# pythoncrazy/jimm

Hardware: NVIDIA H100
Metric: images/sec (higher is better)
Workload: dtype f16

## Files before the change

### jimm_b200/csrc/attention.cu

```cuda
#include <cmath>
#include <type_traits>

#include "common.cuh"
#include "kernels.cuh"

namespace jimm {

__device__ __forceinline__ void cp_async_commit() { asm volatile("cp.async.commit_group;" ::); }
template <int N>
__device__ __forceinline__ void cp_async_wait() { asm volatile("cp.async.wait_group %0;" ::"n"(N)); }

template <typename T>
__device__ __forceinline__ uint32_t pack_pair(float a, float b) {
  if constexpr (std::is_same<T, __half>::value) {
    __half2 h = __floats2half2_rn(a, b);
    return *reinterpret_cast<uint32_t*>(&h);
  } else {
    __nv_bfloat162 h = __floats2bfloat162_rn(a, b);
    return *reinterpret_cast<uint32_t*>(&h);
  }
}

static constexpr int QT = 64;
static constexpr int KT = 64;

template <int DP>
struct HeadTile {
  static_assert(DP % 16 == 0 && DP >= 16 && DP <= 128, "padded head width");
  static constexpr int ROWB = DP * 2;
  static constexpr int SW = ROWB % 128 == 0 ? 128 : ROWB % 64 == 0 ? 64 : 32;
  static constexpr int NB = ROWB / SW;
  static constexpr int CH = SW / 16;
  static constexpr int NCH = DP / 8;
  static constexpr int BYTES = QT * ROWB;
  static constexpr int SMEM = 5 * BYTES;
  static __device__ __forceinline__ uint32_t off(uint32_t row, uint32_t ch) {
    const uint32_t blk = ch / CH, cb = ch % CH;
    return blk * (QT * SW) + row * SW + ((cb ^ ((row * SW >> 7) & (CH - 1))) << 4);
  }
  static __device__ __forceinline__ uint64_t kstep(int ks) { return static_cast<uint64_t>(((ks * 32) / SW * (QT * SW) + (ks * 32) % SW) >> 4); }
};

__device__ __forceinline__ void cp_async16_zfill(uint32_t dst, const void* src, uint32_t src_bytes) {
  asm volatile("cp.async.cg.shared.global [%0], [%1], 16, %2;" ::"r"(dst), "l"(src), "r"(src_bytes));
}

template <typename T, int DP>
__device__ __forceinline__ void load_tile(uint32_t smem_base, const T* __restrict__ gbase, size_t ld, int s0, int S, int d, int tid) {
  using L = HeadTile<DP>;
#pragma unroll
  for (int i = 0; i < L::NCH * QT / 128; ++i) {
    const uint32_t c = tid + i * 128;
    const uint32_t row = c / L::NCH, ch = c % L::NCH;
    int s = s0 + static_cast<int>(row);
    s = s < S ? s : S - 1;
    const bool in = static_cast<int>(ch * 8) < d;
    const T* src = gbase + static_cast<size_t>(s) * ld + (in ? ch * 8 : 0);
    cp_async16_zfill(smem_base + L::off(row, ch), src, in ? 16u : 0u);
  }
}

template <int BYTES, bool STATIC = (BYTES <= 48 * 1024)>
struct AttnSmem {
  static __device__ __forceinline__ uint8_t* get() {
    __shared__ __align__(1024) uint8_t smem[BYTES];
    return smem;
  }
};
template <int BYTES>
struct AttnSmem<BYTES, false> {
  static __device__ __forceinline__ uint8_t* get() {
    extern __shared__ uint8_t smem_raw[];
    return reinterpret_cast<uint8_t*>((reinterpret_cast<uintptr_t>(smem_raw) + 1023) & ~static_cast<uintptr_t>(1023));
  }
};

template <bool PACKED>
__device__ __forceinline__ void sample_rows(int b, int S_arg, const int* __restrict__ seq_off, size_t& row0, int& S) {
  if constexpr (PACKED) {
    row0 = static_cast<size_t>(seq_off[b]);
    S = seq_off[b + 1] - seq_off[b];
  } else {
    row0 = static_cast<size_t>(b) * S_arg;
    S = S_arg;
  }
}

template <typename T, int DP>
__device__ __forceinline__ void score_tile(float (&s)[8][4], uint64_t qdesc, uint32_t sK) {
  using L = HeadTile<DP>;
  constexpr bool BF16 = std::is_same<T, __nv_bfloat16>::value;
  float (&s_acc)[32] = reinterpret_cast<float (&)[32]>(s);
  const uint64_t kdesc = make_wgmma_desc<L::SW>(sK, 16);
#pragma unroll
  for (int i = 0; i < 32; ++i) s_acc[i] = 0.f;
  wgmma_fence_operands(s_acc);
  wgmma_fence();
#pragma unroll
  for (int ks = 0; ks < DP / 16; ++ks)
    wgmma_m64n64k16_ss<BF16>(s_acc, qdesc + L::kstep(ks), kdesc + L::kstep(ks), ks != 0 ? 1u : 0u);
  wgmma_commit();
  wgmma_wait<0>();
  wgmma_fence_operands(s_acc);
}

template <bool CAUSAL>
__device__ __forceinline__ void mask_tile(float (&s)[8][4], int k0, int q0, int row_lo, int t4, int S) {
  if ((k0 + KT > S) || (CAUSAL && (k0 + KT - 1 > q0))) {
#pragma unroll
    for (int nt = 0; nt < 8; ++nt) {
#pragma unroll
      for (int e = 0; e < 4; ++e) {
        const int key = k0 + nt * 8 + t4 * 2 + (e & 1);
        const int qrow = row_lo + (e >> 1) * 8;
        const bool ok = key < S && (!CAUSAL || key <= qrow);
        if (!ok) s[nt][e] = -INFINITY;
      }
    }
  }
}

__device__ __forceinline__ float2 softmax_step(float (&s)[8][4], float (&m_run)[2], float (&l_run)[2], float scale_log2) {
  float mx[2] = {-INFINITY, -INFINITY};
#pragma unroll
  for (int nt = 0; nt < 8; ++nt) {
    mx[0] = fmaxf(mx[0], fmaxf(s[nt][0], s[nt][1]));
    mx[1] = fmaxf(mx[1], fmaxf(s[nt][2], s[nt][3]));
  }
  float alpha[2], moff[2];
#pragma unroll
  for (int r = 0; r < 2; ++r) {
    mx[r] = fmaxf(mx[r], __shfl_xor_sync(0xffffffffu, mx[r], 1));
    mx[r] = fmaxf(mx[r], __shfl_xor_sync(0xffffffffu, mx[r], 2));
    const float mnew = fmaxf(m_run[r], mx[r]);
    const float muse = (mnew == -INFINITY) ? 0.f : mnew;
    alpha[r] = exp2f((m_run[r] - muse) * scale_log2);
    m_run[r] = mnew;
    moff[r] = muse * scale_log2;
    l_run[r] *= alpha[r];
  }
#pragma unroll
  for (int nt = 0; nt < 8; ++nt) {
    s[nt][0] = exp2f(s[nt][0] * scale_log2 - moff[0]);
    s[nt][1] = exp2f(s[nt][1] * scale_log2 - moff[0]);
    s[nt][2] = exp2f(s[nt][2] * scale_log2 - moff[1]);
    s[nt][3] = exp2f(s[nt][3] * scale_log2 - moff[1]);
    l_run[0] += s[nt][0] + s[nt][1];
    l_run[1] += s[nt][2] + s[nt][3];
  }
  return make_float2(alpha[0], alpha[1]);
}

__device__ __forceinline__ float row_inv_sum(float l) {
  l += __shfl_xor_sync(0xffffffffu, l, 1);
  l += __shfl_xor_sync(0xffffffffu, l, 2);
  return 1.0f / l;
}

template <typename T, typename OutT, bool CAUSAL, int DP, bool PACKED = false>
__global__ void __launch_bounds__(128)
attention_kernel(const T* __restrict__ qkv, OutT* __restrict__ out, int S_arg, int H, int d, float scale_log2, int reverse,
                 const int* __restrict__ seq_off) {
  using L = HeadTile<DP>;
  uint8_t* smem = AttnSmem<L::SMEM>::get();
  const int tid = threadIdx.x, warp = tid >> 5, lane = tid & 31;
  const int qt = blockIdx.x, h = blockIdx.y, b = reverse ? static_cast<int>(gridDim.z) - 1 - static_cast<int>(blockIdx.z) : static_cast<int>(blockIdx.z);
  const int D = H * d;
  const size_t ld = static_cast<size_t>(3) * D;
  if constexpr (PACKED) {
    pdl_launch_dependents();
    pdl_wait();
  }
  size_t row0;
  int S;
  sample_rows<PACKED>(b, S_arg, seq_off, row0, S);
  if (PACKED && qt * QT >= S) return;
  const T* base = qkv + row0 * ld + h * d;
  const T* gq = base;
  const T* gk = base + D;
  const T* gv = base + 2 * D;
  const uint32_t sQ = smem_u32(smem);
  const uint32_t sK0 = sQ + L::BYTES;
  const uint32_t sV0 = sK0 + 2 * L::BYTES;
  const int q0 = qt * QT;
  if constexpr (!PACKED) {
    pdl_launch_dependents();
    pdl_wait();
  }
  int n_kv = (S + KT - 1) / KT;
  if (CAUSAL) n_kv = min(n_kv, qt + 1);

  load_tile<T, DP>(sQ, gq, ld, q0, S, d, tid);
  load_tile<T, DP>(sK0, gk, ld, 0, S, d, tid);
  load_tile<T, DP>(sV0, gv, ld, 0, S, d, tid);
  cp_async_commit();

  constexpr bool BF16 = std::is_same<T, __nv_bfloat16>::value;
  const uint64_t qdesc = make_wgmma_desc<L::SW>(sQ, 16);
  float o[DP / 8][4];
#pragma unroll
  for (int i = 0; i < DP / 8; ++i)
#pragma unroll
    for (int j = 0; j < 4; ++j) o[i][j] = 0.f;
  float m_run[2] = {-INFINITY, -INFINITY}, l_run[2] = {0.f, 0.f};
  const int g = lane >> 2, t4 = lane & 3;
  const int row_lo = q0 + warp * 16 + g;

  for (int j = 0; j < n_kv; ++j) {
    const int buf = j & 1;
    if (j + 1 < n_kv) {
      load_tile<T, DP>(sK0 + (buf ^ 1) * L::BYTES, gk, ld, (j + 1) * KT, S, d, tid);
      load_tile<T, DP>(sV0 + (buf ^ 1) * L::BYTES, gv, ld, (j + 1) * KT, S, d, tid);
      cp_async_commit();
      cp_async_wait<1>();
    } else {
      cp_async_wait<0>();
    }
    fence_proxy_async_smem();
    __syncthreads();
    const uint32_t sK = sK0 + buf * L::BYTES, sV = sV0 + buf * L::BYTES;

    float s[8][4];
    score_tile<T, DP>(s, qdesc, sK);
    mask_tile<CAUSAL>(s, j * KT, q0, row_lo, t4, S);
    const float2 alpha = softmax_step(s, m_run, l_run, scale_log2);
#pragma unroll
    for (int nt = 0; nt < DP / 8; ++nt) {
      o[nt][0] *= alpha.x; o[nt][1] *= alpha.x;
      o[nt][2] *= alpha.y; o[nt][3] *= alpha.y;
    }
    uint32_t pf[4][4];
#pragma unroll
    for (int kk = 0; kk < 4; ++kk) {
      pf[kk][0] = pack_pair<T>(s[2 * kk][0], s[2 * kk][1]);
      pf[kk][1] = pack_pair<T>(s[2 * kk][2], s[2 * kk][3]);
      pf[kk][2] = pack_pair<T>(s[2 * kk + 1][0], s[2 * kk + 1][1]);
      pf[kk][3] = pack_pair<T>(s[2 * kk + 1][2], s[2 * kk + 1][3]);
    }
    float (&o_acc)[DP / 2] = reinterpret_cast<float (&)[DP / 2]>(o);
    const uint64_t vdesc = make_wgmma_desc<L::SW>(sV, L::NB > 1 ? QT * L::SW : 16);
    wgmma_fence_operands(o_acc);
    wgmma_fence();
#pragma unroll
    for (int kk = 0; kk < 4; ++kk) wgmma_m64nNk16_rs<BF16, DP>(o_acc, pf[kk], vdesc + static_cast<uint64_t>(kk * (16 * L::SW >> 4)));
    wgmma_commit();
    wgmma_wait<0>();
    wgmma_fence_operands(o_acc);
    __syncthreads();
  }

  const float inv[2] = {row_inv_sum(l_run[0]), row_inv_sum(l_run[1])};
  OutT* obase = out + row0 * D + h * d;
  if constexpr (sizeof(OutT) == 2) {
    uint8_t* sq = smem;
#pragma unroll
    for (int nt = 0; nt < DP / 8; ++nt) {
#pragma unroll
      for (int r = 0; r < 2; ++r) {
        const int row = warp * 16 + g + r * 8;
        const int ch = nt;
        const uint32_t v = pack_pair<OutT>(o[nt][2 * r] * inv[r], o[nt][2 * r + 1] * inv[r]);
        *reinterpret_cast<uint32_t*>(sq + L::off(row, ch) + t4 * 4) = v;
      }
    }
    __syncwarp();
#pragma unroll
    for (int i = 0; i < L::NCH / 2; ++i) {
      const uint32_t c = i * 32 + lane;
      const int row = warp * 16 + static_cast<int>(c / L::NCH), ch = static_cast<int>(c % L::NCH);
      const int srow = q0 + row;
      if (srow < S && ch * 8 < d) {
        const uint4 v = *reinterpret_cast<const uint4*>(sq + L::off(row, ch));
        *reinterpret_cast<uint4*>(obase + static_cast<size_t>(srow) * D + ch * 8) = v;
      }
    }
  } else {
#pragma unroll
    for (int nt = 0; nt < DP / 8; ++nt) {
      if (nt * 8 >= d) break;
#pragma unroll
      for (int r = 0; r < 2; ++r) {
        const int srow = row_lo + r * 8;
        if (srow < S) {
          float2 v = make_float2(o[nt][2 * r] * inv[r], o[nt][2 * r + 1] * inv[r]);
          if constexpr (std::is_same<OutT, tf32_t>::value) v = make_float2(round_tf32(v.x), round_tf32(v.y));
          *reinterpret_cast<float2*>(reinterpret_cast<float*>(obase) + static_cast<size_t>(srow) * D + nt * 8 + t4 * 2) = v;
        }
      }
    }
  }
}

static int padded_head_dim(int d) { return d <= 16 ? 16 : d <= 32 ? 32 : d <= 64 ? 64 : d <= 80 ? 80 : d <= 96 ? 96 : 128; }

static float attn_scale_log2(int d) { return static_cast<float>(1.0 / std::sqrt(static_cast<double>(d))) * 1.4426950408889634f; }

template <typename F>
static int attn_variant(int d, int causal, const int* seq_off, F&& f) {
  auto at_width = [&](auto c, auto p) -> int {
    switch (padded_head_dim(d)) {
      case 16: return f(c, std::integral_constant<int, 16>{}, p);
      case 32: return f(c, std::integral_constant<int, 32>{}, p);
      case 64: return f(c, std::integral_constant<int, 64>{}, p);
      case 80: return f(c, std::integral_constant<int, 80>{}, p);
      case 96: return f(c, std::integral_constant<int, 96>{}, p);
      default: return f(c, std::integral_constant<int, 128>{}, p);
    }
  };
  if (seq_off && causal) return at_width(std::true_type{}, std::true_type{});
  if (seq_off) return at_width(std::false_type{}, std::true_type{});
  if (causal) return at_width(std::true_type{}, std::false_type{});
  return at_width(std::false_type{}, std::false_type{});
}

template <auto Kernel, int SMEM, typename... Args>
static int attn_launch_k(int B, int S, int H, cudaStream_t stream, Args... args) {
  constexpr int dyn = SMEM <= 48 * 1024 ? 0 : SMEM + 1024;
  if constexpr (dyn > 0) {
    if (int rc = smem_opt_in<Kernel>(dyn)) return rc;
  }
  JIMM_CUDA_CHECK(launch_k(Kernel, dim3((S + QT - 1) / QT, H, B), dim3(128), dyn, stream, 1, true, args...));
  note_launch();
  return 0;
}

template <typename T>
struct Type {
  using type = T;
};
template <typename F>
static int io_out_dispatch(const char* name, int io_type, int out_type, F&& f) {
  if (io_type == DT_F16 && out_type == DT_F16) return f(Type<__half>{}, Type<__half>{});
  if (io_type == DT_F16 && out_type == DT_F32) return f(Type<__half>{}, Type<float>{});
  if (io_type == DT_F16 && out_type == DT_TF32) return f(Type<__half>{}, Type<tf32_t>{});
  if (io_type == DT_BF16 && out_type == DT_BF16) return f(Type<__nv_bfloat16>{}, Type<__nv_bfloat16>{});
  if (io_type == DT_BF16 && out_type == DT_F32) return f(Type<__nv_bfloat16>{}, Type<float>{});
  set_last_error("%s: unsupported dtype combination io=%d out=%d", name, io_type, out_type);
  return -1;
}

static bool head_dim_ok(int d) { return d >= 8 && d <= 128 && d % 8 == 0; }

static int attn_dispatch(const void* qkv, int io_type, void* out, int out_type, int B, int S, int H, int head_dim, int causal, cudaStream_t stream,
                         int reverse, const int* seq_off) {
  if (!head_dim_ok(head_dim)) { set_last_error("attention: head_dim %d is not a multiple of 8 in [8, 128]", head_dim); return -1; }
  if (B <= 0 || S <= 0) return 0;
  if (B > 65535 || H > 65535) { set_last_error("attention: grid too large (B=%d H=%d)", B, H); return -1; }
  return io_out_dispatch("attention", io_type, out_type, [&](auto io, auto o) {
    using T = typename decltype(io)::type;
    using OutT = typename decltype(o)::type;
    return attn_variant(head_dim, causal, seq_off, [&](auto c, auto dp, auto p) {
      constexpr int DP = decltype(dp)::value;
      return attn_launch_k<attention_kernel<T, OutT, decltype(c)::value, DP, decltype(p)::value>, HeadTile<DP>::SMEM>(
          B, S, H, stream, static_cast<const T*>(qkv), static_cast<OutT*>(out), S, H, head_dim, attn_scale_log2(head_dim), reverse, seq_off);
    });
  });
}

int attention_run(const void* qkv, int io_type, void* out, int out_type, int B, int S, int H, int head_dim, int causal, cudaStream_t stream, int reverse) {
  return attn_dispatch(qkv, io_type, out, out_type, B, S, H, head_dim, causal, stream, reverse, nullptr);
}

int attention_packed_run(const void* qkv, int io_type, void* out, int out_type, const int* seq_off, int B, int max_S, int H, int head_dim,
                         int causal, cudaStream_t stream, int reverse) {
  if (!seq_off) { set_last_error("attention_packed: null seq_off"); return -1; }
  return attn_dispatch(qkv, io_type, out, out_type, B, max_S, H, head_dim, causal, stream, reverse, seq_off);
}

template <int DP, int OUTB>
struct ProbsSmem {
  static constexpr int STAGE_LD = OUTB == 4 ? 72 : 36;
  static constexpr int STAGE = QT * STAGE_LD * 4;
  static constexpr int BYTES = 3 * HeadTile<DP>::BYTES + STAGE;
};

template <typename T, typename OutT, bool CAUSAL, int DP, bool PACKED>
__global__ void __launch_bounds__(128)
attn_probs_kernel(const T* __restrict__ qkv, OutT* __restrict__ out, int S_arg, int H, int d, float scale_log2, const int* __restrict__ seq_off) {
  using L = HeadTile<DP>;
  using PS = ProbsSmem<DP, static_cast<int>(sizeof(OutT))>;
  uint8_t* smem = AttnSmem<PS::BYTES>::get();
  const int tid = threadIdx.x, warp = tid >> 5, lane = tid & 31;
  const int qt = blockIdx.x, h = blockIdx.y, b = blockIdx.z;
  const int D = H * d;
  const size_t ld = static_cast<size_t>(3) * D;
  uint32_t* stage = reinterpret_cast<uint32_t*>(smem + 3 * L::BYTES);
  pdl_launch_dependents();
  pdl_wait();
  size_t row0;
  int S;
  sample_rows<PACKED>(b, S_arg, seq_off, row0, S);
  size_t obase = static_cast<size_t>(b) * H * S_arg * S_arg;
  if constexpr (PACKED) {
    if (qt * QT >= S) return;
    unsigned long long acc = 0;
    for (int j = tid; j < b; j += 128) {
      const unsigned long long n = static_cast<unsigned long long>(seq_off[j + 1] - seq_off[j]);
      acc += n * n;
    }
#pragma unroll
// ... 270 lines not shown
```

### jimm_b200/csrc/common.cuh

```cuda
#pragma once

#include <cuda.h>
#include <cuda_bf16.h>
#include <cuda_fp16.h>
#include <cuda_fp8.h>
#include <cuda_runtime.h>
#include <stdint.h>

#include <atomic>
#include <mutex>
#include <string>

namespace jimm {

void set_last_error(const char* fmt, ...);

#define JIMM_CUDA_CHECK(expr)                                                                   \
  do {                                                                                          \
    cudaError_t _e = (expr);                                                                    \
    if (_e != cudaSuccess) {                                                                    \
      ::jimm::set_last_error("%s:%d: %s -> %s", __FILE__, __LINE__, #expr, cudaGetErrorString(_e)); \
      return -2;                                                                                \
    }                                                                                           \
  } while (0)
// ... 138 lines not shown
          smem_u32(smem_dst)),
      "l"(reinterpret_cast<uint64_t>(m)), "r"(smem_u32(bar)), "r"(c0), "r"(c1)
      : "memory");
}

__device__ __forceinline__ void tma_store_2d(const CUtensorMap* m, uint32_t smem_src, int c0, int c1) {
  asm volatile("cp.async.bulk.tensor.2d.global.shared::cta.bulk_group [%0, {%2, %3}], [%1];" ::"l"(reinterpret_cast<uint64_t>(m)),
               "r"(smem_src), "r"(c0), "r"(c1)
               : "memory");
}
__device__ __forceinline__ void tma_reduce_add_2d(const CUtensorMap* m, uint32_t smem_src, int c0, int c1) {
  asm volatile("cp.reduce.async.bulk.tensor.2d.global.shared::cta.add.tile.bulk_group [%0, {%2, %3}], [%1];" ::"l"(
                   reinterpret_cast<uint64_t>(m)),
               "r"(smem_src), "r"(c0), "r"(c1)
               : "memory");
}
__device__ __forceinline__ void tma_store_3d(const CUtensorMap* m, uint32_t smem_src, int c0, int c1, int c2) {
  asm volatile("cp.async.bulk.tensor.3d.global.shared::cta.bulk_group [%0, {%2, %3, %4}], [%1];" ::"l"(reinterpret_cast<uint64_t>(m)),
               "r"(smem_src), "r"(c0), "r"(c1), "r"(c2)
               : "memory");
}
__device__ __forceinline__ void tma_reduce_add_3d(const CUtensorMap* m, uint32_t smem_src, int c0, int c1, int c2) {
  asm volatile("cp.reduce.async.bulk.tensor.3d.global.shared::cta.add.tile.bulk_group [%0, {%2, %3, %4}], [%1];" ::"l"(
                   reinterpret_cast<uint64_t>(m)),
               "r"(smem_src), "r"(c0), "r"(c1), "r"(c2)
               : "memory");
}
__device__ __forceinline__ void tma_store_commit() { asm volatile("cp.async.bulk.commit_group;" ::: "memory"); }
__device__ __forceinline__ void tma_store_wait_read() { asm volatile("cp.async.bulk.wait_group.read 0;" ::: "memory"); }
__device__ __forceinline__ void tma_store_wait_read1() { asm volatile("cp.async.bulk.wait_group.read 1;" ::: "memory"); }
__device__ __forceinline__ void tma_store_wait_all() { asm volatile("cp.async.bulk.wait_group 0;" ::: "memory"); }

__device__ __forceinline__ uint32_t cluster_ctarank() {
  uint32_t r;
  asm volatile("mov.u32 %0, %%cluster_ctarank;" : "=r"(r));
  return r;
}
__device__ __forceinline__ void cluster_sync_all() {
  asm volatile("barrier.cluster.arrive.release.aligned;\n\tbarrier.cluster.wait.acquire.aligned;" ::: "memory");
}
__device__ __forceinline__ uint32_t mapa_shared(uint32_t local_smem_addr, uint32_t rank) {
  uint32_t r;
  asm volatile("mapa.shared::cluster.u32 %0, %1, %2;" : "=r"(r) : "r"(local_smem_addr), "r"(rank));
  return r;
}
__device__ __forceinline__ void mbar_arrive_cluster(uint32_t cluster_addr) {
  asm volatile("mbarrier.arrive.release.cluster.shared::cluster.b64 _, [%0];" ::"r"(cluster_addr) : "memory");
}
__device__ __forceinline__ uint64_t make_wgmma_desc_sw128(uint32_t smem_addr) {
  uint64_t d = 0;
  d |= static_cast<uint64_t>((smem_addr & 0x3FFFFu) >> 4);
  d |= static_cast<uint64_t>(1) << 16;
  d |= static_cast<uint64_t>(1024 >> 4) << 32;
  d |= static_cast<uint64_t>(1) << 62;
  return d;
}
template <int SW>
__device__ __forceinline__ uint64_t make_wgmma_desc(uint32_t smem_addr, uint32_t lbo) {
  static_assert(SW == 128 || SW == 64 || SW == 32, "swizzle width");
  constexpr uint64_t layout = SW == 128 ? 1 : SW == 64 ? 2 : 3;
  uint64_t d = 0;
  d |= static_cast<uint64_t>((smem_addr & 0x3FFFFu) >> 4);
  d |= static_cast<uint64_t>((lbo >> 4) & 0x3FFFu) << 16;
  d |= static_cast<uint64_t>(8 * SW >> 4) << 32;
  d |= layout << 62;
  return d;
}
__device__ __forceinline__ void wgmma_fence() { asm volatile("wgmma.fence.sync.aligned;" ::: "memory"); }
__device__ __forceinline__ void wgmma_commit() { asm volatile("wgmma.commit_group.sync.aligned;" ::: "memory"); }
template <int N>
__device__ __forceinline__ void wgmma_wait() { asm volatile("wgmma.wait_group.sync.aligned %0;" ::"n"(N) : "memory"); }
template <int R>
__device__ __forceinline__ void wgmma_fence_operands(float (&d)[R]) {
#pragma unroll
  for (int i = 0; i < R; ++i) asm volatile("" : "+f"(d[i])::"memory");
}

#define JIMM_WGMMA_D128                                                                                                                    \
  "{%0, %1, %2, %3, %4, %5, %6, %7, %8, %9, %10, %11, %12, %13, %14, %15, %16, %17, %18, %19, %20, %21, %22, %23, %24, %25, %26, %27, "     \
  "%28, %29, %30, %31, %32, %33, %34, %35, %36, %37, %38, %39, %40, %41, %42, %43, %44, %45, %46, %47, %48, %49, %50, %51, %52, %53, %54, " \
  "%55, %56, %57, %58, %59, %60, %61, %62, %63, %64, %65, %66, %67, %68, %69, %70, %71, %72, %73, %74, %75, %76, %77, %78, %79, %80, %81, " \
  "%82, %83, %84, %85, %86, %87, %88, %89, %90, %91, %92, %93, %94, %95, %96, %97, %98, %99, %100, %101, %102, %103, %104, %105, %106, "   \
  "%107, %108, %109, %110, %111, %112, %113, %114, %115, %116, %117, %118, %119, %120, %121, %122, %123, %124, %125, %126, %127}"
#define JIMM_WGMMA_D8(i) "+f"(d[i]), "+f"(d[i + 1]), "+f"(d[i + 2]), "+f"(d[i + 3]), "+f"(d[i + 4]), "+f"(d[i + 5]), "+f"(d[i + 6]), "+f"(d[i + 7])
#define JIMM_WGMMA_D128_OPERANDS                                                                                                 \
  JIMM_WGMMA_D8(0), JIMM_WGMMA_D8(8), JIMM_WGMMA_D8(16), JIMM_WGMMA_D8(24), JIMM_WGMMA_D8(32), JIMM_WGMMA_D8(40), JIMM_WGMMA_D8(48), \
      JIMM_WGMMA_D8(56), JIMM_WGMMA_D8(64), JIMM_WGMMA_D8(72), JIMM_WGMMA_D8(80), JIMM_WGMMA_D8(88), JIMM_WGMMA_D8(96),             \
      JIMM_WGMMA_D8(104), JIMM_WGMMA_D8(112), JIMM_WGMMA_D8(120)
template <int KIND>
__device__ __forceinline__ void wgmma_m64n256_ss(float (&d)[128], uint64_t adesc, uint64_t bdesc, uint32_t accumulate) {
  if constexpr (KIND == 0) {
    asm volatile("{\n\t.reg .pred p;\n\tsetp.ne.b32 p, %130, 0;\n\t"
                 "wgmma.mma_async.sync.aligned.m64n256k16.f32.f16.f16 " JIMM_WGMMA_D128 ", %128, %129, p, 1, 1, 0, 0;\n\t}"
                 : JIMM_WGMMA_D128_OPERANDS
                 : "l"(adesc), "l"(bdesc), "r"(accumulate));
  } else if constexpr (KIND == 1) {
    asm volatile("{\n\t.reg .pred p;\n\tsetp.ne.b32 p, %130, 0;\n\t"
                 "wgmma.mma_async.sync.aligned.m64n256k16.f32.bf16.bf16 " JIMM_WGMMA_D128 ", %128, %129, p, 1, 1, 0, 0;\n\t}"
                 : JIMM_WGMMA_D128_OPERANDS
                 : "l"(adesc), "l"(bdesc), "r"(accumulate));
  } else {
    asm volatile("{\n\t.reg .pred p;\n\tsetp.ne.b32 p, %130, 0;\n\t"
                 "wgmma.mma_async.sync.aligned.m64n256k8.f32.tf32.tf32 " JIMM_WGMMA_D128 ", %128, %129, p, 1, 1;\n\t}"
                 : JIMM_WGMMA_D128_OPERANDS
                 : "l"(adesc), "l"(bdesc), "r"(accumulate));
  }
}
__device__ __forceinline__ void wgmma_m64n128k32_e4m3_ss(float (&d)[64], uint64_t adesc, uint64_t bdesc, uint32_t accumulate) {
  asm volatile("{\n\t.reg .pred p;\n\tsetp.ne.b32 p, %66, 0;\n\t"
               "wgmma.mma_async.sync.aligned.m64n128k32.f32.e4m3.e4m3 "
               "{%0, %1, %2, %3, %4, %5, %6, %7, %8, %9, %10, %11, %12, %13, %14, %15, %16, %17, %18, %19, %20, %21, %22, %23, %24, %25, "
               "%26, %27, %28, %29, %30, %31, %32, %33, %34, %35, %36, %37, %38, %39, %40, %41, %42, %43, %44, %45, %46, %47, %48, %49, %50, "
               "%51, %52, %53, %54, %55, %56, %57, %58, %59, %60, %61, %62, %63}, %64, %65, p, 1, 1;\n\t}"
               : JIMM_WGMMA_D8(0), JIMM_WGMMA_D8(8), JIMM_WGMMA_D8(16), JIMM_WGMMA_D8(24), JIMM_WGMMA_D8(32), JIMM_WGMMA_D8(40),
                 JIMM_WGMMA_D8(48), JIMM_WGMMA_D8(56)
               : "l"(adesc), "l"(bdesc), "r"(accumulate));
}
#undef JIMM_WGMMA_D128
#undef JIMM_WGMMA_D8
#undef JIMM_WGMMA_D128_OPERANDS

template <int FROM, int TO>
__device__ __forceinline__ void setmaxnreg() {
  static_assert(TO % 8 == 0 && TO >= 24 && TO <= 256, "setmaxnreg takes a multiple of 8 in [24, 256]");
  if constexpr (TO < FROM) asm volatile("setmaxnreg.dec.sync.aligned.u32 %0;" ::"n"(TO));
  else if constexpr (TO > FROM) asm volatile("setmaxnreg.inc.sync.aligned.u32 %0;" ::"n"(TO));
}

template <bool BF16>
__device__ __forceinline__ void wgmma_m64n64k16_ss(float (&d)[32], uint64_t adesc, uint64_t bdesc, uint32_t accumulate) {
  if constexpr (BF16) {
    asm volatile(
        "{\n\t.reg .pred p;\n\t"
        "setp.ne.b32 p, %34, 0;\n\t"
        "wgmma.mma_async.sync.aligned.m64n64k16.f32.bf16.bf16 {%0, %1, %2, %3, %4, %5, %6, %7, %8, %9, %10, %11, %12, %13, %14, %15, %16, %17, %18, %19, %20, %21, %22, %23, %24, %25, %26, %27, %28, %29, %30, %31}, %32, %33, p, 1, 1, 0, 0;\n\t}"
        : "+f"(d[0]), "+f"(d[1]), "+f"(d[2]), "+f"(d[3]), "+f"(d[4]), "+f"(d[5]), "+f"(d[6]), "+f"(d[7]),
          "+f"(d[8]), "+f"(d[9]), "+f"(d[10]), "+f"(d[11]), "+f"(d[12]), "+f"(d[13]), "+f"(d[14]), "+f"(d[15]),
          "+f"(d[16]), "+f"(d[17]), "+f"(d[18]), "+f"(d[19]), "+f"(d[20]), "+f"(d[21]), "+f"(d[22]), "+f"(d[23]),
          "+f"(d[24]), "+f"(d[25]), "+f"(d[26]), "+f"(d[27]), "+f"(d[28]), "+f"(d[29]), "+f"(d[30]), "+f"(d[31])
        : "l"(adesc), "l"(bdesc), "r"(accumulate));
  } else {
    asm volatile(
        "{\n\t.reg .pred p;\n\t"
        "setp.ne.b32 p, %34, 0;\n\t"
        "wgmma.mma_async.sync.aligned.m64n64k16.f32.f16.f16 {%0, %1, %2, %3, %4, %5, %6, %7, %8, %9, %10, %11, %12, %13, %14, %15, %16, %17, %18, %19, %20, %21, %22, %23, %24, %25, %26, %27, %28, %29, %30, %31}, %32, %33, p, 1, 1, 0, 0;\n\t}"
        : "+f"(d[0]), "+f"(d[1]), "+f"(d[2]), "+f"(d[3]), "+f"(d[4]), "+f"(d[5]), "+f"(d[6]), "+f"(d[7]),
          "+f"(d[8]), "+f"(d[9]), "+f"(d[10]), "+f"(d[11]), "+f"(d[12]), "+f"(d[13]), "+f"(d[14]), "+f"(d[15]),
          "+f"(d[16]), "+f"(d[17]), "+f"(d[18]), "+f"(d[19]), "+f"(d[20]), "+f"(d[21]), "+f"(d[22]), "+f"(d[23]),
          "+f"(d[24]), "+f"(d[25]), "+f"(d[26]), "+f"(d[27]), "+f"(d[28]), "+f"(d[29]), "+f"(d[30]), "+f"(d[31])
        : "l"(adesc), "l"(bdesc), "r"(accumulate));
  }
}
template <bool BF16, int N>
__device__ __forceinline__ void wgmma_m64nNk16_rs(float (&d)[N / 2], const uint32_t (&a)[4], uint64_t bdesc) {
  static_assert(N == 16 || N == 32 || N == 64 || N == 80 || N == 96 || N == 128, "no wgmma_m64nNk16_rs wrapper for this N");
  if constexpr (N == 16) {
    if constexpr (BF16) {
      asm volatile(
          "wgmma.mma_async.sync.aligned.m64n16k16.f32.bf16.bf16 {%0, %1, %2, %3, %4, %5, %6, %7}, {%8, %9, %10, %11}, %12, 1, 1, 1, 1;"
          : "+f"(d[0]), "+f"(d[1]), "+f"(d[2]), "+f"(d[3]), "+f"(d[4]), "+f"(d[5]), "+f"(d[6]), "+f"(d[7])
          : "r"(a[0]), "r"(a[1]), "r"(a[2]), "r"(a[3]), "l"(bdesc));
    } else {
      asm volatile(
          "wgmma.mma_async.sync.aligned.m64n16k16.f32.f16.f16 {%0, %1, %2, %3, %4, %5, %6, %7}, {%8, %9, %10, %11}, %12, 1, 1, 1, 1;"
          : "+f"(d[0]), "+f"(d[1]), "+f"(d[2]), "+f"(d[3]), "+f"(d[4]), "+f"(d[5]), "+f"(d[6]), "+f"(d[7])
          : "r"(a[0]), "r"(a[1]), "r"(a[2]), "r"(a[3]), "l"(bdesc));
    }
  } else if constexpr (N == 32) {
    if constexpr (BF16) {
      asm volatile(
          "wgmma.mma_async.sync.aligned.m64n32k16.f32.bf16.bf16 {%0, %1, %2, %3, %4, %5, %6, %7, %8, %9, %10, %11, %12, %13, %14, %15}, {%16, %17, %18, %19}, %20, 1, 1, 1, 1;"
          : "+f"(d[0]), "+f"(d[1]), "+f"(d[2]), "+f"(d[3]), "+f"(d[4]), "+f"(d[5]), "+f"(d[6]), "+f"(d[7]),
            "+f"(d[8]), "+f"(d[9]), "+f"(d[10]), "+f"(d[11]), "+f"(d[12]), "+f"(d[13]), "+f"(d[14]), "+f"(d[15])
          : "r"(a[0]), "r"(a[1]), "r"(a[2]), "r"(a[3]), "l"(bdesc));
    } else {
      asm volatile(
          "wgmma.mma_async.sync.aligned.m64n32k16.f32.f16.f16 {%0, %1, %2, %3, %4, %5, %6, %7, %8, %9, %10, %11, %12, %13, %14, %15}, {%16, %17, %18, %19}, %20, 1, 1, 1, 1;"
          : "+f"(d[0]), "+f"(d[1]), "+f"(d[2]), "+f"(d[3]), "+f"(d[4]), "+f"(d[5]), "+f"(d[6]), "+f"(d[7]),
            "+f"(d[8]), "+f"(d[9]), "+f"(d[10]), "+f"(d[11]), "+f"(d[12]), "+f"(d[13]), "+f"(d[14]), "+f"(d[15])
          : "r"(a[0]), "r"(a[1]), "r"(a[2]), "r"(a[3]), "l"(bdesc));
    }
  } else if constexpr (N == 64) {
    if constexpr (BF16) {
      asm volatile(
          "wgmma.mma_async.sync.aligned.m64n64k16.f32.bf16.bf16 {%0, %1, %2, %3, %4, %5, %6, %7, %8, %9, %10, %11, %12, %13, %14, %15, %16, %17, %18, %19, %20, %21, %22, %23, %24, %25, %26, %27, %28, %29, %30, %31}, {%32, %33, %34, %35}, %36, 1, 1, 1, 1;"
          : "+f"(d[0]), "+f"(d[1]), "+f"(d[2]), "+f"(d[3]), "+f"(d[4]), "+f"(d[5]), "+f"(d[6]), "+f"(d[7]),
            "+f"(d[8]), "+f"(d[9]), "+f"(d[10]), "+f"(d[11]), "+f"(d[12]), "+f"(d[13]), "+f"(d[14]), "+f"(d[15]),
            "+f"(d[16]), "+f"(d[17]), "+f"(d[18]), "+f"(d[19]), "+f"(d[20]), "+f"(d[21]), "+f"(d[22]), "+f"(d[23]),
            "+f"(d[24]), "+f"(d[25]), "+f"(d[26]), "+f"(d[27]), "+f"(d[28]), "+f"(d[29]), "+f"(d[30]), "+f"(d[31])
          : "r"(a[0]), "r"(a[1]), "r"(a[2]), "r"(a[3]), "l"(bdesc));
    } else {
      asm volatile(
          "wgmma.mma_async.sync.aligned.m64n64k16.f32.f16.f16 {%0, %1, %2, %3, %4, %5, %6, %7, %8, %9, %10, %11, %12, %13, %14, %15, %16, %17, %18, %19, %20, %21, %22, %23, %24, %25, %26, %27, %28, %29, %30, %31}, {%32, %33, %34, %35}, %36, 1, 1, 1, 1;"
          : "+f"(d[0]), "+f"(d[1]), "+f"(d[2]), "+f"(d[3]), "+f"(d[4]), "+f"(d[5]), "+f"(d[6]), "+f"(d[7]),
            "+f"(d[8]), "+f"(d[9]), "+f"(d[10]), "+f"(d[11]), "+f"(d[12]), "+f"(d[13]), "+f"(d[14]), "+f"(d[15]),
            "+f"(d[16]), "+f"(d[17]), "+f"(d[18]), "+f"(d[19]), "+f"(d[20]), "+f"(d[21]), "+f"(d[22]), "+f"(d[23]),
            "+f"(d[24]), "+f"(d[25]), "+f"(d[26]), "+f"(d[27]), "+f"(d[28]), "+f"(d[29]), "+f"(d[30]), "+f"(d[31])
          : "r"(a[0]), "r"(a[1]), "r"(a[2]), "r"(a[3]), "l"(bdesc));
    }
  } else if constexpr (N == 80) {
    if constexpr (BF16) {
      asm volatile(
          "wgmma.mma_async.sync.aligned.m64n80k16.f32.bf16.bf16 {%0, %1, %2, %3, %4, %5, %6, %7, %8, %9, %10, %11, %12, %13, %14, %15, %16, %17, %18, %19, %20, %21, %22, %23, %24, %25, %26, %27, %28, %29, %30, %31, %32, %33, %34, %35, %36, %37, %38, %39}, {%40, %41, %42, %43}, %44, 1, 1, 1, 1;"
          : "+f"(d[0]), "+f"(d[1]), "+f"(d[2]), "+f"(d[3]), "+f"(d[4]), "+f"(d[5]), "+f"(d[6]), "+f"(d[7]),
            "+f"(d[8]), "+f"(d[9]), "+f"(d[10]), "+f"(d[11]), "+f"(d[12]), "+f"(d[13]), "+f"(d[14]), "+f"(d[15]),
            "+f"(d[16]), "+f"(d[17]), "+f"(d[18]), "+f"(d[19]), "+f"(d[20]), "+f"(d[21]), "+f"(d[22]), "+f"(d[23]),
            "+f"(d[24]), "+f"(d[25]), "+f"(d[26]), "+f"(d[27]), "+f"(d[28]), "+f"(d[29]), "+f"(d[30]), "+f"(d[31]),
            "+f"(d[32]), "+f"(d[33]), "+f"(d[34]), "+f"(d[35]), "+f"(d[36]), "+f"(d[37]), "+f"(d[38]), "+f"(d[39])
          : "r"(a[0]), "r"(a[1]), "r"(a[2]), "r"(a[3]), "l"(bdesc));
    } else {
      asm volatile(
          "wgmma.mma_async.sync.aligned.m64n80k16.f32.f16.f16 {%0, %1, %2, %3, %4, %5, %6, %7, %8, %9, %10, %11, %12, %13, %14, %15, %16, %17, %18, %19, %20, %21, %22, %23, %24, %25, %26, %27, %28, %29, %30, %31, %32, %33, %34, %35, %36, %37, %38, %39}, {%40, %41, %42, %43}, %44, 1, 1, 1, 1;"
          : "+f"(d[0]), "+f"(d[1]), "+f"(d[2]), "+f"(d[3]), "+f"(d[4]), "+f"(d[5]), "+f"(d[6]), "+f"(d[7]),
            "+f"(d[8]), "+f"(d[9]), "+f"(d[10]), "+f"(d[11]), "+f"(d[12]), "+f"(d[13]), "+f"(d[14]), "+f"(d[15]),
            "+f"(d[16]), "+f"(d[17]), "+f"(d[18]), "+f"(d[19]), "+f"(d[20]), "+f"(d[21]), "+f"(d[22]), "+f"(d[23]),
            "+f"(d[24]), "+f"(d[25]), "+f"(d[26]), "+f"(d[27]), "+f"(d[28]), "+f"(d[29]), "+f"(d[30]), "+f"(d[31]),
            "+f"(d[32]), "+f"(d[33]), "+f"(d[34]), "+f"(d[35]), "+f"(d[36]), "+f"(d[37]), "+f"(d[38]), "+f"(d[39])
          : "r"(a[0]), "r"(a[1]), "r"(a[2]), "r"(a[3]), "l"(bdesc));
    }
  } else if constexpr (N == 96) {
    if constexpr (BF16) {
      asm volatile(
          "wgmma.mma_async.sync.aligned.m64n96k16.f32.bf16.bf16 {%0, %1, %2, %3, %4, %5, %6, %7, %8, %9, %10, %11, %12, %13, %14, %15, %16, %17, %18, %19, %20, %21, %22, %23, %24, %25, %26, %27, %28, %29, %30, %31, %32, %33, %34, %35, %36, %37, %38, %39, %40, %41, %42, %43, %44, %45, %46, %47}, {%48, %49, %50, %51}, %52, 1, 1, 1, 1;"
          : "+f"(d[0]), "+f"(d[1]), "+f"(d[2]), "+f"(d[3]), "+f"(d[4]), "+f"(d[5]), "+f"(d[6]), "+f"(d[7]),
            "+f"(d[8]), "+f"(d[9]), "+f"(d[10]), "+f"(d[11]), "+f"(d[12]), "+f"(d[13]), "+f"(d[14]), "+f"(d[15]),
            "+f"(d[16]), "+f"(d[17]), "+f"(d[18]), "+f"(d[19]), "+f"(d[20]), "+f"(d[21]), "+f"(d[22]), "+f"(d[23]),
            "+f"(d[24]), "+f"(d[25]), "+f"(d[26]), "+f"(d[27]), "+f"(d[28]), "+f"(d[29]), "+f"(d[30]), "+f"(d[31]),
            "+f"(d[32]), "+f"(d[33]), "+f"(d[34]), "+f"(d[35]), "+f"(d[36]), "+f"(d[37]), "+f"(d[38]), "+f"(d[39]),
            "+f"(d[40]), "+f"(d[41]), "+f"(d[42]), "+f"(d[43]), "+f"(d[44]), "+f"(d[45]), "+f"(d[46]), "+f"(d[47])
          : "r"(a[0]), "r"(a[1]), "r"(a[2]), "r"(a[3]), "l"(bdesc));
    } else {
      asm volatile(
          "wgmma.mma_async.sync.aligned.m64n96k16.f32.f16.f16 {%0, %1, %2, %3, %4, %5, %6, %7, %8, %9, %10, %11, %12, %13, %14, %15, %16, %17, %18, %19, %20, %21, %22, %23, %24, %25, %26, %27, %28, %29, %30, %31, %32, %33, %34, %35, %36, %37, %38, %39, %40, %41, %42, %43, %44, %45, %46, %47}, {%48, %49, %50, %51}, %52, 1, 1, 1, 1;"
          : "+f"(d[0]), "+f"(d[1]), "+f"(d[2]), "+f"(d[3]), "+f"(d[4]), "+f"(d[5]), "+f"(d[6]), "+f"(d[7]),
            "+f"(d[8]), "+f"(d[9]), "+f"(d[10]), "+f"(d[11]), "+f"(d[12]), "+f"(d[13]), "+f"(d[14]), "+f"(d[15]),
            "+f"(d[16]), "+f"(d[17]), "+f"(d[18]), "+f"(d[19]), "+f"(d[20]), "+f"(d[21]), "+f"(d[22]), "+f"(d[23]),
            "+f"(d[24]), "+f"(d[25]), "+f"(d[26]), "+f"(d[27]), "+f"(d[28]), "+f"(d[29]), "+f"(d[30]), "+f"(d[31]),
            "+f"(d[32]), "+f"(d[33]), "+f"(d[34]), "+f"(d[35]), "+f"(d[36]), "+f"(d[37]), "+f"(d[38]), "+f"(d[39]),
            "+f"(d[40]), "+f"(d[41]), "+f"(d[42]), "+f"(d[43]), "+f"(d[44]), "+f"(d[45]), "+f"(d[46]), "+f"(d[47])
          : "r"(a[0]), "r"(a[1]), "r"(a[2]), "r"(a[3]), "l"(bdesc));
    }
  } else if constexpr (N == 128) {
    if constexpr (BF16) {
      asm volatile(
          "wgmma.mma_async.sync.aligned.m64n128k16.f32.bf16.bf16 {%0, %1, %2, %3, %4, %5, %6, %7, %8, %9, %10, %11, %12, %13, %14, %15, %16, %17, %18, %19, %20, %21, %22, %23, %24, %25, %26, %27, %28, %29, %30, %31, %32, %33, %34, %35, %36, %37, %38, %39, %40, %41, %42, %43, %44, %45, %46, %47, %48, %49, %50, %51, %52, %53, %54, %55, %56, %57, %58, %59, %60, %61, %62, %63}, {%64, %65, %66, %67}, %68, 1, 1, 1, 1;"
          : "+f"(d[0]), "+f"(d[1]), "+f"(d[2]), "+f"(d[3]), "+f"(d[4]), "+f"(d[5]), "+f"(d[6]), "+f"(d[7]),
            "+f"(d[8]), "+f"(d[9]), "+f"(d[10]), "+f"(d[11]), "+f"(d[12]), "+f"(d[13]), "+f"(d[14]), "+f"(d[15]),
            "+f"(d[16]), "+f"(d[17]), "+f"(d[18]), "+f"(d[19]), "+f"(d[20]), "+f"(d[21]), "+f"(d[22]), "+f"(d[23]),
            "+f"(d[24]), "+f"(d[25]), "+f"(d[26]), "+f"(d[27]), "+f"(d[28]), "+f"(d[29]), "+f"(d[30]), "+f"(d[31]),
            "+f"(d[32]), "+f"(d[33]), "+f"(d[34]), "+f"(d[35]), "+f"(d[36]), "+f"(d[37]), "+f"(d[38]), "+f"(d[39]),
            "+f"(d[40]), "+f"(d[41]), "+f"(d[42]), "+f"(d[43]), "+f"(d[44]), "+f"(d[45]), "+f"(d[46]), "+f"(d[47]),
            "+f"(d[48]), "+f"(d[49]), "+f"(d[50]), "+f"(d[51]), "+f"(d[52]), "+f"(d[53]), "+f"(d[54]), "+f"(d[55]),
            "+f"(d[56]), "+f"(d[57]), "+f"(d[58]), "+f"(d[59]), "+f"(d[60]), "+f"(d[61]), "+f"(d[62]), "+f"(d[63])
          : "r"(a[0]), "r"(a[1]), "r"(a[2]), "r"(a[3]), "l"(bdesc));
    } else {
      asm volatile(
          "wgmma.mma_async.sync.aligned.m64n128k16.f32.f16.f16 {%0, %1, %2, %3, %4, %5, %6, %7, %8, %9, %10, %11, %12, %13, %14, %15, %16, %17, %18, %19, %20, %21, %22, %23, %24, %25, %26, %27, %28, %29, %30, %31, %32, %33, %34, %35, %36, %37, %38, %39, %40, %41, %42, %43, %44, %45, %46, %47, %48, %49, %50, %51, %52, %53, %54, %55, %56, %57, %58, %59, %60, %61, %62, %63}, {%64, %65, %66, %67}, %68, 1, 1, 1, 1;"
          : "+f"(d[0]), "+f"(d[1]), "+f"(d[2]), "+f"(d[3]), "+f"(d[4]), "+f"(d[5]), "+f"(d[6]), "+f"(d[7]),
            "+f"(d[8]), "+f"(d[9]), "+f"(d[10]), "+f"(d[11]), "+f"(d[12]), "+f"(d[13]), "+f"(d[14]), "+f"(d[15]),
            "+f"(d[16]), "+f"(d[17]), "+f"(d[18]), "+f"(d[19]), "+f"(d[20]), "+f"(d[21]), "+f"(d[22]), "+f"(d[23]),
            "+f"(d[24]), "+f"(d[25]), "+f"(d[26]), "+f"(d[27]), "+f"(d[28]), "+f"(d[29]), "+f"(d[30]), "+f"(d[31]),
            "+f"(d[32]), "+f"(d[33]), "+f"(d[34]), "+f"(d[35]), "+f"(d[36]), "+f"(d[37]), "+f"(d[38]), "+f"(d[39]),
            "+f"(d[40]), "+f"(d[41]), "+f"(d[42]), "+f"(d[43]), "+f"(d[44]), "+f"(d[45]), "+f"(d[46]), "+f"(d[47]),
            "+f"(d[48]), "+f"(d[49]), "+f"(d[50]), "+f"(d[51]), "+f"(d[52]), "+f"(d[53]), "+f"(d[54]), "+f"(d[55]),
            "+f"(d[56]), "+f"(d[57]), "+f"(d[58]), "+f"(d[59]), "+f"(d[60]), "+f"(d[61]), "+f"(d[62]), "+f"(d[63])
          : "r"(a[0]), "r"(a[1]), "r"(a[2]), "r"(a[3]), "l"(bdesc));
    }
  }
}

__device__ __forceinline__ void named_bar_sync(int id, int nthreads) { asm volatile("bar.sync %0, %1;" ::"r"(id), "r"(nthreads) : "memory"); }

__device__ __forceinline__ float tanh_fast(float x) {
  float y;
  asm("tanh.approx.f32 %0, %1;" : "=f"(y) : "f"(x));
  return y;
}
__device__ __forceinline__ float ex2_fast(float x) {
  float y;
  asm("ex2.approx.ftz.f32 %0, %1;" : "=f"(y) : "f"(x));
  return y;
}
__device__ __forceinline__ float rcp_fast(float x) {
  float y;
  asm("rcp.approx.ftz.f32 %0, %1;" : "=f"(y) : "f"(x));
  return y;
}
__device__ __forceinline__ float gelu_tanh(float x) {
  const float c0 = -2.0f * 0.7978845608028654f * 1.4426950408889634f;
  const float c1 = c0 * 0.044715f;
  const float z = x * fmaf(x * x, c1, c0);
  return x * rcp_fast(1.0f + ex2_fast(z));
}
__device__ __forceinline__ float quick_gelu(float x) { return x * rcp_fast(1.0f + ex2_fast(x * (-1.702f * 1.4426950408889634f))); }

__device__ __forceinline__ float warp_sum(float v) {
#pragma unroll
  for (int o = 16; o > 0; o >>= 1) v += __shfl_xor_sync(0xffffffffu, v, o);
  return v;
}
__device__ __forceinline__ float warp_max(float v) {
#pragma unroll
  for (int o = 16; o > 0; o >>= 1) v = fmaxf(v, __shfl_xor_sync(0xffffffffu, v, o));
  return v;
}

// ... 54 lines not shown
```

Baseline: 12150.

## Shrink attention MMA width on partial key tiles and raise occupancy hint

Adds narrower score and PV wgmma variants (N=16/32) and dispatches to them when the last key tile has few valid keys, skipping tensor-core work on padded keys. For ViT sequence lengths like 197, the tail tile holds only a handful of keys, so most of that tile's work is wasted. Out-of-range rows are now zero-filled instead of clamped to the last row. The launch bounds also request 5 blocks per SM for non-causal small-head kernels, which may force register spills. Runtime branching over three template instantiations grows code size.

```diff
diff --git a/jimm_b200/csrc/attention.cu b/jimm_b200/csrc/attention.cu
--- a/jimm_b200/csrc/attention.cu
+++ b/jimm_b200/csrc/attention.cu
@@ -52,10 +52,9 @@
   for (int i = 0; i < L::NCH * QT / 128; ++i) {
     const uint32_t c = tid + i * 128;
     const uint32_t row = c / L::NCH, ch = c % L::NCH;
-    int s = s0 + static_cast<int>(row);
-    s = s < S ? s : S - 1;
-    const bool in = static_cast<int>(ch * 8) < d;
-    const T* src = gbase + static_cast<size_t>(s) * ld + (in ? ch * 8 : 0);
+    const int s = s0 + static_cast<int>(row);
+    const bool in = s < S && static_cast<int>(ch * 8) < d;
+    const T* src = in ? gbase + static_cast<size_t>(s) * ld + ch * 8 : gbase;
     cp_async16_zfill(smem_base + L::off(row, ch), src, in ? 16u : 0u);
   }
 }
@@ -86,22 +85,23 @@
   }
 }
 
-template <typename T, int DP>
+template <typename T, int DP, int NN = KT>
 __device__ __forceinline__ void score_tile(float (&s)[8][4], uint64_t qdesc, uint32_t sK) {
   using L = HeadTile<DP>;
   constexpr bool BF16 = std::is_same<T, __nv_bfloat16>::value;
   float (&s_acc)[32] = reinterpret_cast<float (&)[32]>(s);
+  float (&s_mma)[NN / 2] = reinterpret_cast<float (&)[NN / 2]>(s);
   const uint64_t kdesc = make_wgmma_desc<L::SW>(sK, 16);
 #pragma unroll
   for (int i = 0; i < 32; ++i) s_acc[i] = 0.f;
-  wgmma_fence_operands(s_acc);
+  wgmma_fence_operands(s_mma);
   wgmma_fence();
 #pragma unroll
   for (int ks = 0; ks < DP / 16; ++ks)
-    wgmma_m64n64k16_ss<BF16>(s_acc, qdesc + L::kstep(ks), kdesc + L::kstep(ks), ks != 0 ? 1u : 0u);
+    wgmma_m64nNk16_ss<BF16, NN>(s_mma, qdesc + L::kstep(ks), kdesc + L::kstep(ks), ks != 0 ? 1u : 0u);
   wgmma_commit();
   wgmma_wait<0>();
-  wgmma_fence_operands(s_acc);
+  wgmma_fence_operands(s_mma);
 }
 
 template <bool CAUSAL>
@@ -120,10 +120,11 @@
   }
 }
 
+template <int NT = 8>
 __device__ __forceinline__ float2 softmax_step(float (&s)[8][4], float (&m_run)[2], float (&l_run)[2], float scale_log2) {
   float mx[2] = {-INFINITY, -INFINITY};
 #pragma unroll
-  for (int nt = 0; nt < 8; ++nt) {
+  for (int nt = 0; nt < NT; ++nt) {
     mx[0] = fmaxf(mx[0], fmaxf(s[nt][0], s[nt][1]));
     mx[1] = fmaxf(mx[1], fmaxf(s[nt][2], s[nt][3]));
   }
@@ -140,7 +141,7 @@
     l_run[r] *= alpha[r];
   }
 #pragma unroll
-  for (int nt = 0; nt < 8; ++nt) {
+  for (int nt = 0; nt < NT; ++nt) {
     s[nt][0] = exp2f(s[nt][0] * scale_log2 - moff[0]);
     s[nt][1] = exp2f(s[nt][1] * scale_log2 - moff[0]);
     s[nt][2] = exp2f(s[nt][2] * scale_log2 - moff[1]);
@@ -148,6 +149,8 @@
     l_run[0] += s[nt][0] + s[nt][1];
     l_run[1] += s[nt][2] + s[nt][3];
   }
+#pragma unroll
+  for (int nt = NT; nt < 8; ++nt) s[nt][0] = s[nt][1] = s[nt][2] = s[nt][3] = 0.f;
   return make_float2(alpha[0], alpha[1]);
 }
 
@@ -157,8 +160,52 @@
   return 1.0f / l;
 }
 
+template <typename T, int DP, bool CAUSAL, int NN>
+__device__ __forceinline__ void flash_tile_n(float (&o)[DP / 8][4], float (&m_run)[2], float (&l_run)[2], uint64_t qdesc, uint32_t sK,
+                                             uint32_t sV, int k0, int nk, int q0, int row_lo, int t4, int S, float scale_log2) {
+  using L = HeadTile<DP>;
+  constexpr bool BF16 = std::is_same<T, __nv_bfloat16>::value;
+  constexpr int KK = NN / 16;
+  float s[8][4];
+  score_tile<T, DP, NN>(s, qdesc, sK);
+  mask_tile<CAUSAL>(s, k0, q0, row_lo, t4, S);
+  const float2 alpha = softmax_step<NN / 8>(s, m_run, l_run, scale_log2);
+#pragma unroll
+  for (int nt = 0; nt < DP / 8; ++nt) {
+    o[nt][0] *= alpha.x; o[nt][1] *= alpha.x;
+    o[nt][2] *= alpha.y; o[nt][3] *= alpha.y;
+  }
+  uint32_t pf[KK][4];
+#pragma unroll
+  for (int kk = 0; kk < KK; ++kk) {
+    pf[kk][0] = pack_pair<T>(s[2 * kk][0], s[2 * kk][1]);
+    pf[kk][1] = pack_pair<T>(s[2 * kk][2], s[2 * kk][3]);
+    pf[kk][2] = pack_pair<T>(s[2 * kk + 1][0], s[2 * kk + 1][1]);
+    pf[kk][3] = pack_pair<T>(s[2 * kk + 1][2], s[2 * kk + 1][3]);
+  }
+  float (&o_acc)[DP / 2] = reinterpret_cast<float (&)[DP / 2]>(o);
+  const uint64_t vdesc = make_wgmma_desc<L::SW>(sV, L::NB > 1 ? QT * L::SW : 16);
+  wgmma_fence_operands(o_acc);
+  wgmma_fence();
+#pragma unroll
+  for (int kk = 0; kk < KK; ++kk)
+    if (NN == KT || kk * 16 < nk) wgmma_m64nNk16_rs<BF16, DP>(o_acc, pf[kk], vdesc + static_cast<uint64_t>(kk * (16 * L::SW >> 4)));
+  wgmma_commit();
+  wgmma_wait<0>();
+  wgmma_fence_operands(o_acc);
+}
+
+template <typename T, int DP, bool CAUSAL>
+__device__ __forceinline__ void flash_tile(float (&o)[DP / 8][4], float (&m_run)[2], float (&l_run)[2], uint64_t qdesc, uint32_t sK, uint32_t sV,
+                                           int k0, int q0, int row_lo, int t4, int S, float scale_log2) {
+  const int nk = min(KT, S - k0);
+  if (nk > 32) flash_tile_n<T, DP, CAUSAL, 64>(o, m_run, l_run, qdesc, sK, sV, k0, nk, q0, row_lo, t4, S, scale_log2);
+  else if (nk > 16) flash_tile_n<T, DP, CAUSAL, 32>(o, m_run, l_run, qdesc, sK, sV, k0, nk, q0, row_lo, t4, S, scale_log2);
+  else flash_tile_n<T, DP, CAUSAL, 16>(o, m_run, l_run, qdesc, sK, sV, k0, nk, q0, row_lo, t4, S, scale_log2);
+}
+
 template <typename T, typename OutT, bool CAUSAL, int DP, bool PACKED = false>
-__global__ void __launch_bounds__(128)
+__global__ void __launch_bounds__(128, !CAUSAL && DP <= 64 ? 5 : 1)
 attention_kernel(const T* __restrict__ qkv, OutT* __restrict__ out, int S_arg, int H, int d, float scale_log2, int reverse,
                  const int* __restrict__ seq_off) {
   using L = HeadTile<DP>;
@@ -195,7 +242,6 @@
   load_tile<T, DP>(sV0, gv, ld, 0, S, d, tid);
   cp_async_commit();
 
-  constexpr bool BF16 = std::is_same<T, __nv_bfloat16>::value;
   const uint64_t qdesc = make_wgmma_desc<L::SW>(sQ, 16);
   float o[DP / 8][4];
 #pragma unroll
@@ -218,34 +264,7 @@
     }
     fence_proxy_async_smem();
     __syncthreads();
-    const uint32_t sK = sK0 + buf * L::BYTES, sV = sV0 + buf * L::BYTES;
-
-    float s[8][4];
-    score_tile<T, DP>(s, qdesc, sK);
-    mask_tile<CAUSAL>(s, j * KT, q0, row_lo, t4, S);
-    const float2 alpha = softmax_step(s, m_run, l_run, scale_log2);
-#pragma unroll
-    for (int nt = 0; nt < DP / 8; ++nt) {
-      o[nt][0] *= alpha.x; o[nt][1] *= alpha.x;
-      o[nt][2] *= alpha.y; o[nt][3] *= alpha.y;
-    }
-    uint32_t pf[4][4];
-#pragma unroll
-    for (int kk = 0; kk < 4; ++kk) {
-      pf[kk][0] = pack_pair<T>(s[2 * kk][0], s[2 * kk][1]);
-      pf[kk][1] = pack_pair<T>(s[2 * kk][2], s[2 * kk][3]);
-      pf[kk][2] = pack_pair<T>(s[2 * kk + 1][0], s[2 * kk + 1][1]);
-      pf[kk][3] = pack_pair<T>(s[2 * kk + 1][2], s[2 * kk + 1][3]);
-    }
-    float (&o_acc)[DP / 2] = reinterpret_cast<float (&)[DP / 2]>(o);
-    const uint64_t vdesc = make_wgmma_desc<L::SW>(sV, L::NB > 1 ? QT * L::SW : 16);
-    wgmma_fence_operands(o_acc);
-    wgmma_fence();
-#pragma unroll
-    for (int kk = 0; kk < 4; ++kk) wgmma_m64nNk16_rs<BF16, DP>(o_acc, pf[kk], vdesc + static_cast<uint64_t>(kk * (16 * L::SW >> 4)));
-    wgmma_commit();
-    wgmma_wait<0>();
-    wgmma_fence_operands(o_acc);
+    flash_tile<T, DP, CAUSAL>(o, m_run, l_run, qdesc, sK0 + buf * L::BYTES, sV0 + buf * L::BYTES, j * KT, q0, row_lo, t4, S, scale_log2);
     __syncthreads();
   }
 
diff --git a/jimm_b200/csrc/common.cuh b/jimm_b200/csrc/common.cuh
--- a/jimm_b200/csrc/common.cuh
+++ b/jimm_b200/csrc/common.cuh
@@ -314,6 +314,46 @@
   }
 }
 template <bool BF16, int N>
+__device__ __forceinline__ void wgmma_m64nNk16_ss(float (&d)[N / 2], uint64_t adesc, uint64_t bdesc, uint32_t accumulate);
+template <>
+__device__ __forceinline__ void wgmma_m64nNk16_ss<false, 16>(float (&d)[8], uint64_t adesc, uint64_t bdesc, uint32_t accumulate) {
+  asm volatile("{\n\t.reg .pred p;\n\tsetp.ne.b32 p, %10, 0;\n\t"
+               "wgmma.mma_async.sync.aligned.m64n16k16.f32.f16.f16 {%0, %1, %2, %3, %4, %5, %6, %7}, %8, %9, p, 1, 1, 0, 0;\n\t}"
+               : "+f"(d[0]), "+f"(d[1]), "+f"(d[2]), "+f"(d[3]), "+f"(d[4]), "+f"(d[5]), "+f"(d[6]), "+f"(d[7])
+               : "l"(adesc), "l"(bdesc), "r"(accumulate));
+}
+template <>
+__device__ __forceinline__ void wgmma_m64nNk16_ss<true, 16>(float (&d)[8], uint64_t adesc, uint64_t bdesc, uint32_t accumulate) {
+  asm volatile("{\n\t.reg .pred p;\n\tsetp.ne.b32 p, %10, 0;\n\t"
+               "wgmma.mma_async.sync.aligned.m64n16k16.f32.bf16.bf16 {%0, %1, %2, %3, %4, %5, %6, %7}, %8, %9, p, 1, 1, 0, 0;\n\t}"
+               : "+f"(d[0]), "+f"(d[1]), "+f"(d[2]), "+f"(d[3]), "+f"(d[4]), "+f"(d[5]), "+f"(d[6]), "+f"(d[7])
+               : "l"(adesc), "l"(bdesc), "r"(accumulate));
+}
+template <>
+__device__ __forceinline__ void wgmma_m64nNk16_ss<false, 32>(float (&d)[16], uint64_t adesc, uint64_t bdesc, uint32_t accumulate) {
+  asm volatile("{\n\t.reg .pred p;\n\tsetp.ne.b32 p, %18, 0;\n\t"
+               "wgmma.mma_async.sync.aligned.m64n32k16.f32.f16.f16 {%0, %1, %2, %3, %4, %5, %6, %7, %8, %9, %10, %11, %12, %13, %14, %15}, %16, %17, p, 1, 1, 0, 0;\n\t}"
+               : "+f"(d[0]), "+f"(d[1]), "+f"(d[2]), "+f"(d[3]), "+f"(d[4]), "+f"(d[5]), "+f"(d[6]), "+f"(d[7]),
+                 "+f"(d[8]), "+f"(d[9]), "+f"(d[10]), "+f"(d[11]), "+f"(d[12]), "+f"(d[13]), "+f"(d[14]), "+f"(d[15])
+               : "l"(adesc), "l"(bdesc), "r"(accumulate));
+}
+template <>
+__device__ __forceinline__ void wgmma_m64nNk16_ss<true, 32>(float (&d)[16], uint64_t adesc, uint64_t bdesc, uint32_t accumulate) {
+  asm volatile("{\n\t.reg .pred p;\n\tsetp.ne.b32 p, %18, 0;\n\t"
+               "wgmma.mma_async.sync.aligned.m64n32k16.f32.bf16.bf16 {%0, %1, %2, %3, %4, %5, %6, %7, %8, %9, %10, %11, %12, %13, %14, %15}, %16, %17, p, 1, 1, 0, 0;\n\t}"
+               : "+f"(d[0]), "+f"(d[1]), "+f"(d[2]), "+f"(d[3]), "+f"(d[4]), "+f"(d[5]), "+f"(d[6]), "+f"(d[7]),
+                 "+f"(d[8]), "+f"(d[9]), "+f"(d[10]), "+f"(d[11]), "+f"(d[12]), "+f"(d[13]), "+f"(d[14]), "+f"(d[15])
+               : "l"(adesc), "l"(bdesc), "r"(accumulate));
+}
+template <>
+__device__ __forceinline__ void wgmma_m64nNk16_ss<false, 64>(float (&d)[32], uint64_t adesc, uint64_t bdesc, uint32_t accumulate) {
+  wgmma_m64n64k16_ss<false>(d, adesc, bdesc, accumulate);
+}
+template <>
+__device__ __forceinline__ void wgmma_m64nNk16_ss<true, 64>(float (&d)[32], uint64_t adesc, uint64_t bdesc, uint32_t accumulate) {
+  wgmma_m64n64k16_ss<true>(d, adesc, bdesc, accumulate);
+}
+template <bool BF16, int N>
 __device__ __forceinline__ void wgmma_m64nNk16_rs(float (&d)[N / 2], const uint32_t (&a)[4], uint64_t bdesc) {
   static_assert(N == 16 || N == 32 || N == 64 || N == 80 || N == 96 || N == 128, "no wgmma_m64nNk16_rs wrapper for this N");
   if constexpr (N == 16) {
```

After: 12200 (median of 6 runs). About the same (+0.4%).
